# thisparticle/scl_slam

Measured on AMD Instinct MI355X. Metric: loop-closure candidates/sec: (scan, keyframe) pairs taken through full-database ARG-MIN detection per second (every pair aligned exactly and bounded by the f16 matrix-core screening; only the survivors get the f64 distance), batches of 16 scans, 10k-keyframe DB per GPU, higher is better.
Workload: dtype f64 results; f16-operand / f32-accumulate MFMA screening + f64 exact pass on the survivors

## Files before the change

### scl_slam_amd/csrc/engine.hip

```cpp
#include "scl_engine.h"

#include <hip/hip_runtime.h>

#include <cfloat>
#include <climits>
#include <chrono>
#include <cmath>
#include <cstdio>
#include <cstdlib>
#include <cstring>
#include <mutex>
#include <new>
#include <string>
#include <atomic>
#include <chrono>
#include <thread>
#include <vector>

#include "db_file.hpp"
#include "engine_internal.hpp"
#include "device_sort.hpp"
#include "plugin_host.hpp"

#ifdef SCL_DIAGNOSTICS
// ... 126 lines not shown
    dev_free(e->d_approx); dev_free(e->d_surv); dev_free(e->d_starts);
    size_t nn = n + n / 2 + 64;
    int rc;
    e->pair_cap = 0;
    if ((rc = dev_alloc(e, &e->d_approx, nn))) return rc;
    if ((rc = dev_alloc(e, &e->d_starts, nn))) return rc;
    if ((rc = dev_alloc(e, &e->d_surv, nn))) return rc;
    if ((rc = dev_alloc(e, &e->d_ring_d2, nn))) return rc;
    if ((rc = dev_alloc(e, &e->d_dist, nn))) return rc;
    if ((rc = dev_alloc(e, &e->d_shift, nn))) return rc;
    if ((rc = dev_alloc(e, &e->d_cand, nn))) return rc;
    e->pair_cap = nn;
    return SCL_OK;
}

int ensure_sets(scl_engine *e, size_t n)
{
    if (n <= e->set_stride && e->pair_cap >= e->set_stride * scl_engine::kScreenSets) return SCL_OK;
    const size_t stride = n + n / 4 + 64;
    int rc = ensure_pairs(e, stride * scl_engine::kScreenSets);
    if (rc) { e->set_stride = 0; return rc; }
    e->set_stride = stride;
    if (e->smask_cap < stride * scl_engine::kScreenSets) {
        dev_free(e->d_smask); e->d_smask = nullptr; e->smask_cap = 0;
        if ((rc = dev_alloc(e, &e->d_smask, stride * scl_engine::kScreenSets))) { e->set_stride = 0; return rc; }
        e->smask_cap = stride * scl_engine::kScreenSets;
    }
    const size_t need = 2 * stride * sc_screen_scratch_floats(db_view(e), e->SR);
    if (need > e->part_cap) {
        dev_free(e->d_part); e->part_cap = 0;
        if ((rc = dev_alloc(e, &e->d_part, need))) { e->set_stride = 0; return rc; }
        e->part_cap = need;
    }
    return SCL_OK;
}

int launch_topk(scl_engine *e, const QueryView &q, int lo, int hi, int k, float eps, hipStream_t on)
{
    hipStream_t s = on ? on : e->stream;
    ProfScope ps(e, P_TOPK, s);
    SCL_HIP(e, launch_ringkey_topk(db_view(e), q.rkey, lo, hi, k, eps, e->d_topk_scratch,
                                   e->d_topk_idx, e->d_topk_d2, s));
    return SCL_OK;
}

}

// ... 379 lines not shown
    if ((rc = dev_alloc(e, &e->d_done_counter, (size_t)4))) return bail(rc);
    if (hipMemset(e->d_done_counter, 0, 16) != hipSuccess) return bail(SCL_ERR_HIP);
    {
        constexpr int NS = scl_engine::kScreenSets;
        if ((rc = dev_alloc(e, &e->d_nsurv, (size_t)NS))) return bail(rc);
        static_assert(NS <= kTminEpsOffset, "the launch's largest bound sits kTminEpsOffset words behind its t_min word");
        if ((rc = dev_alloc(e, &e->d_tmin, (size_t)NS + kTminEpsOffset))) return bail(rc);
        if (hipMemset(e->d_nsurv, 0, sizeof(int) * NS) != hipSuccess) return bail(SCL_ERR_HIP);
        if (hipMemset(e->d_tmin, 0xff, sizeof(unsigned int) * NS) != hipSuccess) return bail(SCL_ERR_HIP);
        if (hipMemset(e->d_tmin + NS, 0, sizeof(unsigned int) * kTminEpsOffset) != hipSuccess) return bail(SCL_ERR_HIP);
        if ((rc = dev_alloc(e, &e->d_surv_part, (size_t)NS * kSurvivorBlocks * kTailRec))) return bail(rc);
        if ((rc = dev_alloc(e, &e->d_surv_done, (size_t)NS))) return bail(rc);
        if (hipMemset(e->d_surv_done, 0, sizeof(unsigned int) * NS) != hipSuccess) return bail(SCL_ERR_HIP);
        if (hipMalloc(&e->d_surv_args, (size_t)8 * NS * kSurvivorArgBytes) != hipSuccess) return bail(SCL_ERR_NOMEM);
        if (hipHostMalloc(&e->h_surv_args, (size_t)8 * NS * kSurvivorArgBytes, hipHostMallocDefault) != hipSuccess) return bail(SCL_ERR_HIP);
        if (hipHostMalloc((void **)&e->h_stream_out, (size_t)2 * NS * 64, hipHostMallocDefault) != hipSuccess) return bail(SCL_ERR_HIP);
        for (auto &ev : e->ev_chunk) if (hipEventCreateWithFlags(&ev, hipEventDisableTiming) != hipSuccess) return bail(SCL_ERR_HIP);
        for (auto &ev : e->ev_k1) if (hipEventCreateWithFlags(&ev, hipEventDisableTiming) != hipSuccess) return bail(SCL_ERR_HIP);
        for (auto &ev : e->ev_sub0) if (hipEventCreateWithFlags(&ev, hipEventDisableTiming) != hipSuccess) return bail(SCL_ERR_HIP);
        if (hipEventCreateWithFlags(&e->ev_align_gate, hipEventDisableTiming) != hipSuccess) return bail(SCL_ERR_HIP);
        {
            int lo_p = 0, hi_p = 0;
            (void)hipDeviceGetStreamPriorityRange(&lo_p, &hi_p);
            const bool wide_grid = e->S == 180 && e->RG == 20;
            if (hipStreamCreateWithPriority(&e->stream_surv, hipStreamNonBlocking, wide_grid ? hi_p : lo_p) != hipSuccess) return bail(SCL_ERR_HIP);
            if (hipStreamCreateWithPriority(&e->stream_queue_place, hipStreamNonBlocking, lo_p) != hipSuccess) return bail(SCL_ERR_HIP);
        }
    }
    if (hipStreamCreateWithFlags(&e->stream_alt, hipStreamNonBlocking) != hipSuccess) return bail(SCL_ERR_HIP);
    if (hipEventCreateWithFlags(&e->ev_db, hipEventDisableTiming) != hipSuccess) return bail(SCL_ERR_HIP);
// ... 49 lines not shown
    dev_free(e->d_smask);
    if (e->d_mat_dist) (void)hipFree(e->d_mat_dist);
    if (e->d_mat_shift) (void)hipFree(e->d_mat_shift);
    if (e->d_rank_key) (void)hipFree(e->d_rank_key);
    if (e->d_rank_pos) (void)hipFree(e->d_rank_pos);
    if (e->d_rank_out) (void)hipFree(e->d_rank_out);
    if (e->h_rank_out) (void)hipHostFree(e->h_rank_out);
    dev_free(e->d_meta_robot); dev_free(e->d_meta_index);
    if (e->h_mat) (void)hipHostFree(e->h_mat);
    for (auto &ev : e->ev_mat_k) if (ev) (void)hipEventDestroy(ev);
    for (auto &ev : e->ev_mat_c) if (ev) (void)hipEventDestroy(ev);
    dev_free(e->d_surv_stats);
    dev_free(e->d_surv_part); dev_free(e->d_surv_done);
    if (e->d_surv_args) (void)hipFree(e->d_surv_args);
    if (e->h_surv_args) (void)hipHostFree(e->h_surv_args);
    if (e->h_stream_out) (void)hipHostFree(e->h_stream_out);
    for (auto ev : e->ev_chunk) if (ev) (void)hipEventDestroy(ev);
    if (e->stream_surv) { (void)hipStreamSynchronize(e->stream_surv); (void)hipStreamDestroy(e->stream_surv); }
    if (e->stream_queue_place) (void)hipStreamDestroy(e->stream_queue_place);
    for (auto ev : e->ev_k1) if (ev) (void)hipEventDestroy(ev);
    for (auto ev : e->ev_sub0) if (ev) (void)hipEventDestroy(ev);
    if (e->ev_align_gate) (void)hipEventDestroy(e->ev_align_gate);
    dev_free(e->d_topk_scratch); dev_free(e->d_topk_idx); dev_free(e->d_topk_d2); dev_free(e->d_out3);
    dev_free(e->d_blk_part); dev_free(e->d_done_counter);
    if (e->ev_db) (void)hipEventDestroy(e->ev_db);
    if (e->stream_alt) { (void)hipStreamSynchronize(e->stream_alt); (void)hipStreamDestroy(e->stream_alt); }
    if (e->h_pinned) (void)hipHostFree(e->h_pinned);
    if (e->h_out3) (void)hipHostFree(e->h_out3);
    if (e->ev_call) (void)hipEventDestroy(e->ev_call);
    for (int i = 0; i < scl_engine::kSlots; ++i) if (e->ev_done[i]) (void)hipEventDestroy(e->ev_done[i]);
// ... 1538 lines not shown
```

### scl_slam_amd/csrc/engine_internal.hpp

```cpp
#pragma once

#include "scl_engine.h"

#include <hip/hip_runtime.h>

#include <chrono>
#include <climits>
#include <initializer_list>
#include <mutex>
#include <string>
#include <vector>

#include "icp.hpp"
#include "kernels.hpp"
#include "pcm.hpp"

namespace scl {

enum ProfKind { P_SC = 0, P_TOPK, P_ARGMIN, P_MAKESC, P_INGEST, P_ICPNN, P_ICPRED, P_COUNT };

struct PendingEvent { hipEvent_t start, stop; int kind; int launches = 1; };

struct ShardedFront;

// ... 39 lines not shown
    unsigned char *d_pbuf[3] = {nullptr, nullptr, nullptr}; size_t pbuf_cap = 0;
    static constexpr int kCopyStreams = 4;
    hipStream_t stream_copy = nullptr;
    hipStream_t stream_copy_x[kCopyStreams - 1] = {nullptr, nullptr, nullptr};
    hipEvent_t ev_copied[kCopyStreams][3] = {}, ev_consumed[3] = {nullptr, nullptr, nullptr};
    std::vector<void *> host_allocs;
    double *d_dist = nullptr; int *d_shift = nullptr; int *d_cand = nullptr; float *d_ring_d2 = nullptr; size_t pair_cap = 0;
#ifndef SCL_SCREEN_SETS
#define SCL_SCREEN_SETS 256
#endif
    static constexpr int kScreenSets = SCL_SCREEN_SETS;
    float *d_approx = nullptr; int *d_starts = nullptr; int *d_surv = nullptr;
    unsigned int *d_smask = nullptr; size_t smask_cap = 0;
    float *d_part = nullptr; size_t part_cap = 0;
    int *d_nsurv = nullptr; unsigned int *d_tmin = nullptr;
    unsigned long long *d_align_fallbacks = nullptr; uint64_t align_pairs = 0;
    unsigned long long *d_surv_stats = nullptr;
    size_t set_stride = 0;
    unsigned long long *d_surv_part = nullptr; unsigned int *d_surv_done = nullptr;
    void *d_surv_args = nullptr; void *h_surv_args = nullptr; unsigned surv_arg_tick = 0;
    double *h_stream_out = nullptr;
    hipEvent_t ev_chunk[2] = {nullptr, nullptr};
    bool exact_heavy = false;
    hipEvent_t ev_sub0[2] = {nullptr, nullptr};
    hipStream_t stream_surv = nullptr;
    hipEvent_t ev_k1[2] = {nullptr, nullptr};
    hipEvent_t ev_align_gate = nullptr;
    hipStream_t stream_queue_place = nullptr;
    bool screen = false;
    bool in_single_fallback = false;
// ... 43 lines not shown

struct ProfScope {
    scl_engine *e; int kind; hipStream_t s; hipEvent_t start = nullptr, stop = nullptr;
    ProfScope(scl_engine *e_, int kind_, hipStream_t s_ = nullptr);
    bool active() const { return start && stop; }
    ~ProfScope();
};
void collect_profile(scl_engine *e);
int sync(scl_engine *e);
hipError_t wait_event_polled(hipEvent_t ev, std::chrono::microseconds budget, bool relax);
void drain_keeping_error(scl_engine *e, const hipStream_t *streams, int n);
inline void drain_keeping_error(scl_engine *e, std::initializer_list<hipStream_t> streams) { drain_keeping_error(e, streams.begin(), (int)streams.size()); }
DbView db_view(const scl_engine *e);
int query_view(const scl_engine *e, int query, QueryView *q);
int ensure_pairs(scl_engine *e, size_t n);
int ensure_sets(scl_engine *e, size_t n);
int launch_topk(scl_engine *e, const QueryView &q, int lo, int hi, int k, float eps, hipStream_t on = nullptr);

template <class T> void dev_free(T *&p) { if (p) { (void)hipFree(p); p = nullptr; } }

constexpr int kQueryOutOfRange = -1, kQueryNotStaged = -2;
inline int query_slot(const scl_engine *e, int query, int n_db)
{
    if (query >= 0) return query < n_db ? query : kQueryOutOfRange;
    const int j = -1 - query;
    return j < e->stage_rows && e->staged[(size_t)j] ? e->cap + j : kQueryNotStaged;
}

inline int clamp_range(int &lo, int &hi, int n_db)
{
    if (lo < 0) lo = 0;
// ... 89 lines not shown
```

### scl_slam_amd/csrc/kernels.hpp

```cpp
#pragma once

#include <hip/hip_runtime.h>
#include <stdint.h>

#include <stdlib.h>

namespace scl {

#ifdef SCL_DIAGNOSTICS
inline int scl_lab_int(const char *name, int dflt) { const char *e = getenv(name); return e ? atoi(e) : dflt; }
inline bool scl_lab_is(const char *name, const char *value) { const char *e = getenv(name); if (!e) return false; while (*value) if (*e++ != *value++) return false; return true; }
#else
constexpr int scl_lab_int(const char *, int dflt) { return dflt; }
constexpr bool scl_lab_is(const char *, const char *) { return false; }
#endif

constexpr double kBigDist = 10000000.0;
constexpr int kTminEpsOffset = 256;
constexpr int hdesc_sector(int RG) { return ((RG * 8 + 63) / 64) * 8; }
constexpr int hkey_halfs(int S) { return ((S + 31) / 32) * 32; }
constexpr int hkey_store_halfs(int S) { return hkey_halfs(S) + 8; }
constexpr int hkey_row_halfs(int S) { return 2 * hkey_halfs(S) + 8; }
constexpr int halign_P(int S) { return S % 8 == 0 ? 8 : (S % 4 == 0 ? 4 : 0); }
constexpr int halign_CP(int S) { return ((S + 8 + 31) / 32) * 32; }
// ... 119 lines not shown
    int k; float exclude_eps; int *topk_idx; float *topk_d2;
    float *part;
    bool no_ring_metric;
};
bool sc_screen_supported(const struct DbView &db, int SR);
bool sc_screen_is_wide(const struct DbView &db, int SR);
float sc_screen_eps();
int sc_screen_max_batch(const struct DbView &db, int SR);
size_t sc_screen_scratch_floats(const struct DbView &db, int SR);
constexpr int kScreenAlign = 1, kScreenProducts = 2;
hipError_t launch_sc_screen_batch(const struct DbView &db, const ScreenBatch &sb, int SR, int align_filter, int num_cu, hipStream_t stream,
                                  int phases = kScreenAlign | kScreenProducts, const ScreenBatch *next = nullptr);
bool sc_screen_pairs(const struct DbView &db, int SR);
hipError_t launch_sc_screen_pair(const struct DbView &db, const ScreenBatch &sb0, const ScreenBatch &sb1, int SR, int align_filter, int num_cu,
                                 hipStream_t stream, const ScreenBatch *next0, const ScreenBatch *next1);
hipError_t launch_sc_select_batch(const ScreenBatch &sb, hipStream_t stream);
constexpr int kSurvivorBlocks = 2;
constexpr int kSurvivorArgBytes = 384;
constexpr int kMaxSurvivorQueries = 128;
struct SurvivorPass {
    int nq;
    int slot[kMaxSurvivorQueries], base[kMaxSurvivorQueries], n[kMaxSurvivorQueries], buf[kMaxSurvivorQueries];
    double *out3[kMaxSurvivorQueries];
    size_t pair_stride;
    const float *approx; int *survivors; unsigned int *t_min; double *out_dist; int *out_shift;
    const float *ring_d2; int k; float exclude_eps; int *topk_idx; float *topk_d2;
    unsigned long long *blk_part; unsigned int *done_counter;
    unsigned long long *surv_stats;
    void *d_args; void *h_args;
    int ring_from_keys;
// ... 62 lines not shown
```

### scl_slam_amd/csrc/sc_screen.hip

```cpp
#include <atomic>
#include <type_traits>

#include "align_exact.hpp"
#include "device_common.hpp"
#include "kernels.hpp"

namespace scl {

namespace {

typedef _Float16 h4 __attribute__((ext_vector_type(4)));
typedef _Float16 h8 __attribute__((ext_vector_type(8)));
typedef float f4v __attribute__((ext_vector_type(4)));
typedef float f2 __attribute__((ext_vector_type(2)));
typedef unsigned int u32x4 __attribute__((ext_vector_type(4)));
typedef u32x4 __attribute__((aligned(8))) u32x4_a8;

struct ScreenArgs {
    const double *vkey;
    const uint2 *hdesc; const unsigned int *kmask;
    const double *q_vkey; const float *q_rkey;
    const uint2 *q_hdesc; const unsigned int *q_kmask;
    const _Float16 *hkey; const _Float16 *q_hkey; int hkw;
    const float4 *rkey4; int rk_cap;
// ... 1738 lines not shown
            sc_align2_role<S, W>(ta.nb[0], ta.halign, ta.u_lo, ta.u_n, wg, wt, tile);
            sc_align2_role<S, W>(ta.nb[1], ta.halign, ta.u_lo, ta.u_n, wg, wt, tile);
        }
#endif
        else sc_align2_role<S, W>(ta.nb[0], ta.halign, ta.u_lo, ta.u_n, wg, wt, tile);
        return;
    }
    int qi, chunk;
    const int nq0 = ta.fin[0].prod.nq;
    if (!finish_block_of(b - ta.align_blocks, nq0 + ta.fin[1].prod.nq, ta.chunks_max, qi, chunk)) return;
    const int set = qi < nq0 ? 0 : 1;
    if (chunk >= ta.chunks[set]) return;
    sc_screen2_finish_body<RG, S, W, MASKS, D2>(ta.fin[set], qi - (set ? nq0 : 0), chunk);
}

static bool screen_second_form()
{
    static const int form = [] { const char *e = getenv("SCL_SCREEN_FORM"); return e ? atoi(e) : 2; }();
    return form != 1;
}
static bool screen_pair_enabled()
{
    static const int on = [] { const char *e = getenv("SCL_SCREEN_PAIR"); return e ? atoi(e) : 1; }();
    return on != 0;
}
static int screen_tail_pair()
{
    static const int v = [] { const char *e = getenv("SCL_TAIL_PAIR"); return e ? atoi(e) : 1; }();
    return v;
}
// ... 16 lines not shown
    ab->vkey = db.vkey; ab->rkey = db.rkey; ab->hdesc = db.hdesc; ab->kmask = db.kmask; ab->rkey4 = db.rkey4; ab->hkey = db.hkey; ab->hkw = hkey_row_halfs(db.S);
    ab->starts = sb.starts; ab->approx = sb.approx; ab->ring_d2 = sb.ring_d2; ab->t_min = sb.t_min; ab->fallbacks = sb.align_fallbacks; ab->smask = sb.smask;
    ab->pair_stride = (unsigned long long)sb.pair_stride;
    ab->S = db.S; ab->R4 = 4 * db.RG; ab->hstride = db.hstride; ab->rk_cap = db.cap; ab->align_filter = align_filter;
    ab->nq = sb.nq;
    int nmax = 0;
    for (int i = 0; i < sb.nq; ++i) {
        if (sb.n[i] <= 0) return -1;
        ab->q[i] = ScreenQuery{sb.slot[i], sb.base[i], sb.n[i], sb.buf[i]};
        nmax = sb.n[i] > nmax ? sb.n[i] : nmax;
    }
    for (int i = sb.nq; i < kMaxScreenBatch; ++i) ab->q[i] = ab->q[0];
    return nmax;
}

struct ScreenPairMate { const ScreenBatch *sb; const ScreenBatch *next; };

template <int RG, int S, int W, int OCC0, int OCC1>
static hipError_t launch_screen_grid(const DbView &db, const ScreenBatch &sb, int align_filter, int num_cu, hipStream_t stream, int phases,
                                     const ScreenBatch *next, const ScreenPairMate *mate = nullptr)
{
    constexpr int RGH = hdesc_rgh(RG);
    ScreenBatchArgs ab{};
    const int nmax = fill_screen_args(db, sb, align_filter, &ab);
    if (nmax < 0) return hipErrorInvalidValue;
    ScreenBatchArgs ab_m{};
    const int nmax_m = mate ? fill_screen_args(db, *mate->sb, align_filter, &ab_m) : 0;
    if (nmax_m < 0) return hipErrorInvalidValue;
    const int ngroups = (nmax + kGroup - 1) / kGroup;
    static_assert(halign_bytes(S) > 0, "alignment image");
    if (db.hstride != hdesc_stride(RG, S) || !sb.starts || !db.halign) return hipErrorInvalidValue;
// ... 97 lines not shown
                    if (e != hipSuccess) return e;
                    attrp.store(true, std::memory_order_release);
                }
                f2_m.prod = ab_m; f2_m.part = mate->sb->part; f2_m.nwg = nwg;
                union_of(*mate->sb, &f2_m.u_lo, &f2_m.u_n);
                Screen2PairArgs fp{};
                fp.prod[0] = ab; fp.prod[1] = ab_m; fp.part[0] = sb.part; fp.part[1] = mate->sb->part; fp.nwg = nwg;
                const int hi0 = f2.u_lo + f2.u_n, hi1 = f2_m.u_lo + f2_m.u_n;
                fp.u_lo = f2.u_lo < f2_m.u_lo ? f2.u_lo : f2_m.u_lo;
                fp.u_n = (hi0 > hi1 ? hi0 : hi1) - fp.u_lo;
                hipLaunchKernelGGL((sc_screen2_kernel<RG, S, W, 2>), dim3(nwg), dim3(S2Cfg<RG, S, W>::WV * kWave), (s2_lds<RG, S, W>()), stream, fp);
            }
        }
        if (!mate) hipLaunchKernelGGL((sc_screen2_kernel<RG, S, W>), dim3(nwg), dim3(S2Cfg<RG, S, W>::WV * kWave), (s2_lds<RG, S, W>()), stream, f2);
        if ((e = hipGetLastError()) != hipSuccess) return e;
        auto launch_tail = [&](const ScreenBatch &sb, const Screen2Args &f2, const int nmax, const ScreenBatch *next) -> hipError_t {
            const bool next_v2 = next && second_form_for(*next);
            const int chunks = (nmax + 255) / 256;
            const dim3 fgrid(finish_blocks(chunks, sb.nq)), ablock(kScreenWaves * kWave);
            if (!next) {
                hipLaunchKernelGGL((sc_screen2_finish_kernel<RG, S, W>), fgrid, dim3(256), 0, stream, f2, chunks);
                return hipGetLastError();
            }
            if (next->nq < 1 || next->nq > kMaxScreenBatch) return hipErrorInvalidValue;
            ScreenBatchArgs nb{};
            const int nmax2 = fill_screen_args(db, *next, align_filter, &nb);
            if (nmax2 < 0) return hipErrorInvalidValue;
            nb.skip_d2 = next_v2 ? 1 : 0;
            int ulo = 0, un = 0, ablocks;
            if (next_v2) {
// ... 94 lines not shown

bool sc_screen_pairs(const DbView &db, int SR)
{
    return sc_screen_supported(db, SR) && !sc_screen_is_wide(db, SR) && screen_second_form() && screen_pair_enabled() && screen_v2_min_env() <= kMaxScreenBatch &&
           scl_lab_int("SCL_SCREEN_VARIANT", 0) == 0 && scl_lab_int("SCL_SCREEN_PROBE", 0) == 0;
}

hipError_t launch_sc_screen_pair(const DbView &db, const ScreenBatch &sb0, const ScreenBatch &sb1, int SR, int align_filter, int num_cu, hipStream_t stream,
                                 const ScreenBatch *next0, const ScreenBatch *next1)
{
    if (!sc_screen_pairs(db, SR) || sb0.nq != kMaxScreenBatch || sb1.nq != kMaxScreenBatch) return hipErrorInvalidValue;
    const ScreenPairMate mate{&sb1, next1};
    return launch_screen_grid<16, 120, 13, 2, 3>(db, sb0, align_filter, num_cu, stream, kScreenProducts, next0, &mate);
}

}

#ifdef S2_STAMP
extern "C" int scl_debug_s2_stamps(unsigned long long *out)
{
    return (int)hipMemcpyFromSymbol(out, HIP_SYMBOL(scl::g_s2_stamps), sizeof(unsigned long long) * 4 * 64);
}
#endif
```

### scl_slam_amd/csrc/screen_host.hip

```cpp
#include "scl_engine.h"

#include <hip/hip_runtime.h>

#include <atomic>
#include <chrono>
#include <mutex>
#include <string>
#include <vector>

#include "engine_internal.hpp"
#include "plugin_host.hpp"
#include "screen_plan.hpp"

using namespace scl;

namespace {

int submit_full_many_locked(scl_engine *e, const int *queries, const int *los, const int *his, int nq, int *tickets);

void screen_batch_pointers(const scl_engine *e, ScreenBatch &sb, bool lists, unsigned long long *surv_stats, unsigned int *smask, float *part)
{
    sb.approx = e->d_approx; sb.starts = e->d_starts; sb.align_fallbacks = e->d_align_fallbacks; sb.ring_d2 = e->d_ring_d2;
    sb.survivors = lists ? e->d_surv : nullptr; sb.n_surv = lists ? e->d_nsurv : nullptr; sb.t_min = e->d_tmin; sb.surv_stats = surv_stats;
    sb.smask = smask; sb.part = part;
    sb.k = e->cfg.num_candidates; sb.exclude_eps = e->cfg.knn_exclude_eps; sb.topk_idx = e->d_topk_idx; sb.topk_d2 = e->d_topk_d2;
}

struct ScreenGroup { const int *qslot, *lo, *n; int nq, set0; int part_half = 0; bool masks = false; bool keys_later = false; };
void fill_screen_batch(scl_engine *e, ScreenBatch &sb, const ScreenGroup &g)
{
    sb.nq = g.nq;
    for (int j = 0; j < g.nq; ++j) { sb.slot[j] = g.qslot[j]; sb.base[j] = g.lo[j]; sb.n[j] = g.n[j]; sb.buf[j] = g.set0 + j; }
    sb.pair_stride = e->set_stride;
    screen_batch_pointers(e, sb, false, nullptr,
                          (g.masks || sc_screen_is_wide(db_view(e), e->SR)) ? e->d_smask : nullptr,
                          e->d_part + (g.part_half ? e->part_cap / 2 : 0));
    sb.no_ring_metric = g.keys_later;
}

int launch_screen_group(scl_engine *e, const ScreenGroup &cur, int phases = kScreenAlign | kScreenProducts,
                        const ScreenGroup *next = nullptr, hipStream_t stream = nullptr)
{
    if (!stream) stream = e->stream;
    ScreenBatch sb{}, nx{};
    fill_screen_batch(e, sb, cur);
    const bool has_next = next && next->nq > 0;
    if (has_next) fill_screen_batch(e, nx, *next);
    if (phases & kScreenAlign) for (int j = 0; j < cur.nq; ++j) e->align_pairs += (uint64_t)cur.n[j];
    if (has_next) for (int j = 0; j < next->nq; ++j) e->align_pairs += (uint64_t)next->n[j];
    if ((phases & kScreenAlign) && (phases & kScreenProducts) && has_next) {
        SCL_HIP(e, launch_sc_screen_batch(db_view(e), sb, e->SR, sc_align_filter_enabled(), e->num_cu, stream, kScreenAlign, nullptr));
// ... 11 lines not shown
    g0.part_half = 0; g1.part_half = 1;
    ScreenBatch sb0{}, sb1{}, nx0{}, nx1{};
    fill_screen_batch(e, sb0, g0);
    fill_screen_batch(e, sb1, g1);
    const bool has0 = next0 && next0->nq > 0, has1 = next1 && next1->nq > 0;
    if (has0) fill_screen_batch(e, nx0, *next0);
    if (has1) fill_screen_batch(e, nx1, *next1);
    const ScreenGroup *counted[4] = {align0 ? &g0 : nullptr, align1 ? &g1 : nullptr, has0 ? next0 : nullptr, has1 ? next1 : nullptr};
    for (const ScreenGroup *g : counted)
        if (g) for (int j = 0; j < g->nq; ++j) e->align_pairs += (uint64_t)g->n[j];
    if (align0) SCL_HIP(e, launch_sc_screen_batch(db_view(e), sb0, e->SR, sc_align_filter_enabled(), e->num_cu, stream, kScreenAlign, nullptr));
    if (align1) SCL_HIP(e, launch_sc_screen_batch(db_view(e), sb1, e->SR, sc_align_filter_enabled(), e->num_cu, stream, kScreenAlign, nullptr));
    ProfScope ps(e, P_SC, stream);
    SCL_HIP(e, launch_sc_screen_pair(db_view(e), sb0, sb1, e->SR, sc_align_filter_enabled(), e->num_cu, stream, has0 ? &nx0 : nullptr, has1 ? &nx1 : nullptr));
    if (ps.active()) { for (int j = 0; j < g0.nq; ++j) e->prof.sc_distance_pairs += (uint64_t)g0.n[j] + (uint64_t)g1.n[j]; }
    return SCL_OK;
}

unsigned survivor_arg_region(scl_engine *e) { return e->surv_arg_tick++ & 7u; }
int launch_survivor_pass(scl_engine *e, const int *qslot, const int *lo, const int *n, int nq, int set0, double *const *out3, hipStream_t stream = nullptr,
                         int phases = kSurvivorArgs | kSurvivorKernel, int region_in = -1, bool ring_from_keys = false)
{
    if (!stream) stream = e->stream;
    SurvivorPass sp{};
    sp.nq = nq; sp.ring_from_keys = ring_from_keys ? 1 : 0;
    for (int j = 0; j < nq; ++j) { sp.slot[j] = qslot[j]; sp.base[j] = lo[j]; sp.n[j] = n[j]; sp.buf[j] = set0 + j; sp.out3[j] = out3[j]; }
    sp.pair_stride = e->set_stride;
    sp.approx = e->d_approx; sp.survivors = e->d_surv; sp.t_min = e->d_tmin; sp.out_dist = e->d_dist; sp.out_shift = e->d_shift;
    sp.blk_part = e->d_surv_part; sp.done_counter = e->d_surv_done; sp.surv_stats = e->d_surv_stats;
    sp.ring_d2 = e->d_ring_d2; sp.k = e->cfg.num_candidates; sp.exclude_eps = e->cfg.knn_exclude_eps; sp.topk_idx = e->d_topk_idx; sp.topk_d2 = e->d_topk_d2;
// ... 371 lines not shown
    const int chmax = wide && CH > SCL_WIDE_CHUNK ? SCL_WIDE_CHUNK : CH;
    const int chn = spl >= 1 && spl <= chmax ? (chmax / spl) * spl : chmax;
    struct List { int qslot[CH], qlo[CH], qn[CH], pos[CH], m = 0; };
    struct Chunk { int first = 0, count = 0; int aligned = 0; bool busy = false, small = false; std::vector<int> lo, empty; };
    Chunk ch[2];
    bool sub0_valid[2] = {false, false};
    const bool small_exact = sc_small_exact_supported(db_view(e), e->SR) && (!wide || e->d_smask) && !scl_lab_is("SCL_STREAM_EXACT", "s");
    const bool keys_later = !wide && !small_exact;
    const bool pairs = !wide && sc_screen_pairs(db_view(e), e->SR);
    int nmax = 1;
    for (int i = 0; i < n_queries; ++i) {
        int l = lo[i], h = hi[i];
        const int n = clamp_range(l, h, n0);
        if (n > nmax) nmax = n;
    }
    int rc = ensure_sets(e, (size_t)nmax);
    if (rc) return rc;
    SCL_HIP(e, hipEventRecord(e->ev_align_gate, e->stream));
    SCL_HIP(e, hipStreamWaitEvent(e->stream_surv, e->ev_align_gate, 0));
    auto build = [&](int first, int count, List &L, Chunk *k) -> int {
        L.m = 0;
        for (int i = 0; i < count; ++i) {
            const int slot = query_slot(e, queries[first + i], n0);
            if (slot == kQueryOutOfRange) return fail(e, SCL_ERR_OUT_OF_RANGE, "query slot out of range");
            if (slot == kQueryNotStaged) return fail(e, SCL_ERR_INVALID_ARG, "no staged query");
            int l = lo[first + i], h = hi[first + i];
            const int n = clamp_range(l, h, n0);
            if (k) k->lo[(size_t)i] = l;
            if (n <= 0) continue;
            if (k) k->empty[(size_t)i] = 0;
            L.qslot[L.m] = slot; L.qlo[L.m] = l; L.qn[L.m] = n; L.pos[L.m] = i;
            ++L.m;
        }
        return SCL_OK;
    };
    auto submit = [&](int c, int first, int count, int nfirst, int ncount) -> int {
        Chunk &k = ch[c];
        k.first = first; k.count = count; k.lo.assign((size_t)count, 0); k.empty.assign((size_t)count, 1);
        List cur, nxt;
        if ((rc = build(first, count, cur, &k))) return rc;
        if (ncount > 0 && (rc = build(nfirst, ncount, nxt, nullptr))) return rc;
        double *out3[CH];
        for (int j = 0; j < cur.m; ++j) out3[j] = e->h_stream_out + ((size_t)c * NS + (size_t)cur.pos[j]) * 8;
        const int set0 = c * CH, nset0 = (c ^ 1) * CH;
        k.small = small_exact && !e->exact_heavy;
        const int region = (cur.m > 0 && (k.small || !wide)) ? (int)survivor_arg_region(e) : 0;
        if (cur.m > 0 && (k.small || !wide) && (rc = k.small ? launch_small_exact_chunk(e, cur.qslot, cur.qlo, cur.qn, cur.m, set0, out3, e->stream_surv, kSurvivorArgs, region)
                                                    : launch_survivor_pass(e, cur.qslot, cur.qlo, cur.qn, cur.m, set0, out3, e->stream_surv, kSurvivorArgs, region, keys_later))) return rc;
        if (ncount == 0 && cur.m > 0) SCL_HIP(e, hipEventRecord(e->ev_k1[c], e->stream_surv));
        struct ProfRestore { scl_engine *e; int saved; ~ProfRestore() { e->prof_on = saved; } } prof_restore{e, e->prof_on};
        hipEvent_t span_start = nullptr, span_stop = nullptr;
        int span_groups = 0;
        if (e->prof_on == 3 && cur.m > 0) {
            if ((e->prof_tick++ & 1) == 0) {
                auto get = [&]() { hipEvent_t ev = nullptr; if (!e->event_pool.empty()) { ev = e->event_pool.back(); e->event_pool.pop_back(); } else if (hipEventCreate(&ev) != hipSuccess) ev = nullptr; return ev; };
                span_start = get(); span_stop = get();
                if (span_start && span_stop) (void)hipEventRecord(span_start, e->stream); else { span_start = span_stop = nullptr; }
            }
            e->prof_on = 0;
        }
        auto span_end = [&]() {
            if (!span_start) return;
            (void)hipEventRecord(span_stop, e->stream);
            e->pending.push_back({span_start, span_stop, P_SC, span_groups});
            for (int j = 0; j < cur.m; ++j) e->prof.sc_distance_pairs += (uint64_t)cur.qn[j];
            span_start = nullptr;
        };
        static_assert(kPlanPairGroup == kMaxScreenBatch, "a pair is two full launch groups");
        PlanUnit units[CH];
        int next_aligned = 0;
        const int n_units = plan_chunk(cur.m, ncount > 0 ? nxt.m : 0, spl, pairs, k.aligned, units, &next_aligned);
        auto group_of = [&](const PlanGroup &p) {
            ScreenGroup g{nullptr, nullptr, nullptr, 0, 0};
            const int o = p.off - cur.m;
            if (p.nq > 0) g = o < 0 ? ScreenGroup{cur.qslot + p.off, cur.qlo + p.off, cur.qn + p.off, p.nq, set0 + p.off} : ScreenGroup{nxt.qslot + o, nxt.qlo + o, nxt.qn + o, p.nq, nset0 + o};
            g.keys_later = keys_later;
            return g;
        };
        for (int i = 0; i < n_units; ++i) {
            const PlanUnit &u = units[i];
            const ScreenGroup g0 = group_of(u.g0), g1 = group_of(u.g1), n0 = group_of(u.n0), n1 = group_of(u.n1);
            if (u.over > 0) {
                if (ch[c ^ 1].busy) SCL_HIP(e, hipStreamWaitEvent(e->stream, (wide && sub0_valid[c ^ 1] && u.over <= kWideExactBatch) ? e->ev_sub0[c ^ 1] : e->ev_chunk[c ^ 1], 0));
            }
            if (g1.nq > 0) rc = launch_screen_pair_group(e, g0, g1, u.align0, u.align1, n0.nq > 0 ? &n0 : nullptr, n1.nq > 0 ? &n1 : nullptr);
            else rc = launch_screen_group(e, g0, u.align0 ? (kScreenAlign | kScreenProducts) : kScreenProducts, n0.nq > 0 ? &n0 : nullptr);
            if (rc) return rc;
            ++span_groups;
        }
        span_end();
        hipStream_t xs = ncount > 0 ? e->stream_surv : e->stream;
        if (ncount > 0) {
            SCL_HIP(e, hipEventRecord(e->ev_k1[c], e->stream));
            SCL_HIP(e, hipStreamWaitEvent(e->stream_surv, e->ev_k1[c], 0));
        } else if (cur.m > 0) {
// ... 241 lines not shown
```

### scl_slam_amd/csrc/screen_plan.hpp

```cpp
#pragma once

namespace scl {

constexpr int kPlanPairGroup = 16;

struct PlanGroup { int off, nq; };

struct PlanUnit {
    PlanGroup g0, g1;
    PlanGroup n0, n1;
    bool align0, align1;
    int over;
};

inline int plan_chunk(int cur_m, int nxt_m, int spl, bool pairs, int aligned_in, PlanUnit *units, int *next_aligned)
{
    const int all_m = cur_m + nxt_m;
    auto group_at = [&](int off) {
        const int end = off < cur_m ? cur_m : all_m;
        if (off >= end) return PlanGroup{0, 0};
        return PlanGroup{off, end - off < spl ? end - off : spl};
    };
    auto pair_at = [&](int off) { return pairs && group_at(off).nq == kPlanPairGroup && group_at(off + kPlanPairGroup).nq == kPlanPairGroup &&
                                         (off + 2 * kPlanPairGroup <= cur_m || off >= cur_m); };
// ... 8 lines not shown
        if (end >= aligned_to) {
            u.n0 = group_at(end);
            if (pair && pair_at(end)) u.n1 = group_at(end + u.n0.nq);
        }
        const int reach = end + u.n0.nq + u.n1.nq;
        u.over = (reach > cur_m && u.n0.nq > 0) ? reach - cur_m : 0;
        u.align0 = g >= aligned_to;
        u.align1 = pair && g + u.g0.nq >= aligned_to;
        if (reach > aligned_to) aligned_to = reach;
        g = end;
    }
    *next_aligned = aligned_to > cur_m ? aligned_to - cur_m : 0;
    return n_units;
}

}
```

Measured before the change: 2.998 billion.

## Batch screen tails of several pair units into one joint run-tail launch

Adds a run planner that groups up to four consecutive full pair units. It launches only their products kernels, then fires a single tail kernel that does the finish work for all sets of the run plus the next groups' alignment. The tail arguments are staged into a ring of pinned host regions and copied on the survivor stream, gated by an event. The aim is fewer small tail launches and better CU fill in the finish and align phase. The cost is an extra partials scratch buffer per run, more host planning, and a cross-stream dependency on the argument copy.

```diff
diff --git a/scl_slam_amd/csrc/engine.hip b/scl_slam_amd/csrc/engine.hip
--- a/scl_slam_amd/csrc/engine.hip
+++ b/scl_slam_amd/csrc/engine.hip
@@ -164,10 +164,11 @@
     return SCL_OK;
 }
 
-int ensure_sets(scl_engine *e, size_t n)
-{
-    if (n <= e->set_stride && e->pair_cap >= e->set_stride * scl_engine::kScreenSets) return SCL_OK;
-    const size_t stride = n + n / 4 + 64;
+int ensure_sets(scl_engine *e, size_t n, int run_pairs)
+{
+    auto run_floats = [&](size_t stride) { return run_pairs > 1 ? (size_t)(2 * run_pairs) * stride * sc_screen_scratch_floats(db_view(e), e->SR) : (size_t)0; };
+    if (n <= e->set_stride && e->pair_cap >= e->set_stride * scl_engine::kScreenSets && e->part_run_cap >= run_floats(e->set_stride)) return SCL_OK;
+    const size_t stride = n <= e->set_stride ? e->set_stride : n + n / 4 + 64;
     int rc = ensure_pairs(e, stride * scl_engine::kScreenSets);
     if (rc) { e->set_stride = 0; return rc; }
     e->set_stride = stride;
@@ -181,6 +182,11 @@
         dev_free(e->d_part); e->part_cap = 0;
         if ((rc = dev_alloc(e, &e->d_part, need))) { e->set_stride = 0; return rc; }
         e->part_cap = need;
+    }
+    if (run_floats(stride) > e->part_run_cap) {
+        dev_free(e->d_part_run); e->part_run_cap = 0;
+        if ((rc = dev_alloc(e, &e->d_part_run, run_floats(stride)))) { e->set_stride = 0; return rc; }
+        e->part_run_cap = run_floats(stride);
     }
     return SCL_OK;
 }
@@ -590,6 +596,9 @@
         if (hipMemset(e->d_surv_done, 0, sizeof(unsigned int) * NS) != hipSuccess) return bail(SCL_ERR_HIP);
         if (hipMalloc(&e->d_surv_args, (size_t)8 * NS * kSurvivorArgBytes) != hipSuccess) return bail(SCL_ERR_NOMEM);
         if (hipHostMalloc(&e->h_surv_args, (size_t)8 * NS * kSurvivorArgBytes, hipHostMallocDefault) != hipSuccess) return bail(SCL_ERR_HIP);
+        if (hipMalloc(&e->d_run_args, (size_t)scl_engine::kRunArgRegions * kScreenRunArgBytes) != hipSuccess) return bail(SCL_ERR_NOMEM);
+        if (hipHostMalloc(&e->h_run_args, (size_t)scl_engine::kRunArgRegions * kScreenRunArgBytes, hipHostMallocDefault) != hipSuccess) return bail(SCL_ERR_HIP);
+        for (auto &ev : e->ev_run_args) if (hipEventCreateWithFlags(&ev, hipEventDisableTiming) != hipSuccess) return bail(SCL_ERR_HIP);
         if (hipHostMalloc((void **)&e->h_stream_out, (size_t)2 * NS * 64, hipHostMallocDefault) != hipSuccess) return bail(SCL_ERR_HIP);
         for (auto &ev : e->ev_chunk) if (hipEventCreateWithFlags(&ev, hipEventDisableTiming) != hipSuccess) return bail(SCL_ERR_HIP);
         for (auto &ev : e->ev_k1) if (hipEventCreateWithFlags(&ev, hipEventDisableTiming) != hipSuccess) return bail(SCL_ERR_HIP);
@@ -669,6 +678,10 @@
     dev_free(e->d_surv_part); dev_free(e->d_surv_done);
     if (e->d_surv_args) (void)hipFree(e->d_surv_args);
     if (e->h_surv_args) (void)hipHostFree(e->h_surv_args);
+    dev_free(e->d_part_run);
+    if (e->d_run_args) (void)hipFree(e->d_run_args);
+    if (e->h_run_args) (void)hipHostFree(e->h_run_args);
+    for (auto &ev : e->ev_run_args) if (ev) (void)hipEventDestroy(ev);
     if (e->h_stream_out) (void)hipHostFree(e->h_stream_out);
     for (auto ev : e->ev_chunk) if (ev) (void)hipEventDestroy(ev);
     if (e->stream_surv) { (void)hipStreamSynchronize(e->stream_surv); (void)hipStreamDestroy(e->stream_surv); }
diff --git a/scl_slam_amd/csrc/engine_internal.hpp b/scl_slam_amd/csrc/engine_internal.hpp
--- a/scl_slam_amd/csrc/engine_internal.hpp
+++ b/scl_slam_amd/csrc/engine_internal.hpp
@@ -77,6 +77,10 @@
     unsigned int *d_smask = nullptr; size_t smask_cap = 0;
     float *d_part = nullptr; size_t part_cap = 0;
     int *d_nsurv = nullptr; unsigned int *d_tmin = nullptr;
+    float *d_part_run = nullptr; size_t part_run_cap = 0;
+    static constexpr int kRunArgRegions = 16;
+    void *d_run_args = nullptr; void *h_run_args = nullptr; unsigned run_arg_tick = 0;
+    hipEvent_t ev_run_args[2] = {nullptr, nullptr};
     unsigned long long *d_align_fallbacks = nullptr; uint64_t align_pairs = 0;
     unsigned long long *d_surv_stats = nullptr;
     size_t set_stride = 0;
@@ -150,7 +154,7 @@
 DbView db_view(const scl_engine *e);
 int query_view(const scl_engine *e, int query, QueryView *q);
 int ensure_pairs(scl_engine *e, size_t n);
-int ensure_sets(scl_engine *e, size_t n);
+int ensure_sets(scl_engine *e, size_t n, int run_pairs = 1);
 int launch_topk(scl_engine *e, const QueryView &q, int lo, int hi, int k, float eps, hipStream_t on = nullptr);
 
 template <class T> void dev_free(T *&p) { if (p) { (void)hipFree(p); p = nullptr; } }
diff --git a/scl_slam_amd/csrc/kernels.hpp b/scl_slam_amd/csrc/kernels.hpp
--- a/scl_slam_amd/csrc/kernels.hpp
+++ b/scl_slam_amd/csrc/kernels.hpp
@@ -157,6 +157,14 @@
 bool sc_screen_pairs(const struct DbView &db, int SR);
 hipError_t launch_sc_screen_pair(const struct DbView &db, const ScreenBatch &sb0, const ScreenBatch &sb1, int SR, int align_filter, int num_cu,
                                  hipStream_t stream, const ScreenBatch *next0, const ScreenBatch *next1);
+constexpr int kScreenRunPairs = 4, kScreenRunSets = 2 * kScreenRunPairs;
+constexpr size_t kScreenRunArgBytes = 12 * 1024;
+int sc_screen_tail_run(const struct DbView &db, int SR);
+hipError_t launch_sc_screen_pair_products(const struct DbView &db, const ScreenBatch &sb0, const ScreenBatch &sb1, int SR, int align_filter, int num_cu,
+                                          hipStream_t stream);
+struct ScreenRunTail { int n_fin, n_al; const ScreenBatch *fin[kScreenRunSets]; const ScreenBatch *al[kScreenRunSets]; };
+hipError_t fill_sc_screen_run_tail(const struct DbView &db, const ScreenRunTail &rt, int SR, int align_filter, int num_cu, void *h_args, unsigned int *grid);
+hipError_t launch_sc_screen_run_tail(const void *d_args, unsigned int grid, hipStream_t stream);
 hipError_t launch_sc_select_batch(const ScreenBatch &sb, hipStream_t stream);
 constexpr int kSurvivorBlocks = 2;
 constexpr int kSurvivorArgBytes = 384;
diff --git a/scl_slam_amd/csrc/sc_screen.hip b/scl_slam_amd/csrc/sc_screen.hip
--- a/scl_slam_amd/csrc/sc_screen.hip
+++ b/scl_slam_amd/csrc/sc_screen.hip
@@ -1,4 +1,5 @@
 #include <atomic>
+#include <new>
 #include <type_traits>
 
 #include "align_exact.hpp"
@@ -1776,6 +1777,43 @@
     sc_screen2_finish_body<RG, S, W, MASKS, D2>(ta.fin[set], qi - (set ? nq0 : 0), chunk);
 }
 
+struct TailRunArgs {
+    Screen2Args fin[kScreenRunSets];
+    ScreenBatchArgs nb[kScreenRunSets];
+    const unsigned char *halign;
+    int n_fin_scans;
+    int chunks[kScreenRunSets], chunks_max;
+    int n_items;
+    int u_lo[kScreenRunPairs], u_n[kScreenRunPairs], ablocks[kScreenRunPairs];
+    int align_blocks;
+};
+static_assert(sizeof(TailRunArgs) <= kScreenRunArgBytes, "argument region of a run's tail");
+
+template <int RG, int S, int W, bool MASKS, bool D2>
+__global__ __launch_bounds__(kScreenWaves * kWave, 3) void sc_screen2_tail_run_kernel(const TailRunArgs *__restrict__ ta_global)
+{
+    extern __shared__ __attribute__((aligned(16))) unsigned char smem_tailr[];
+    typedef const TailRunArgs __attribute__((address_space(4))) *ConstArgs;
+    const ConstArgs ta = (ConstArgs)ta_global;
+    const int b = (int)blockIdx.x;
+    const int align_blocks = ta->align_blocks;
+    if (b < align_blocks) {
+        const int n_items = ta->n_items;
+        const int s = b >> 3, r = s / n_items, item = s - r * n_items, wb = 8 * r + (b & 7);
+        const int ab = ta->ablocks[item];
+        if (wb >= ab) return;
+        const int wave = __builtin_amdgcn_readfirstlane((int)(threadIdx.x >> 6));
+        sc_align2_pair_role<S, W>((const ScreenBatchArgs *)(ta->nb + 2 * item), ta->halign, ta->u_lo[item], ta->u_n[item], wb * kScreenWaves + wave, ab * kScreenWaves,
+                                  smem_tailr + (size_t)wave * Align2Cfg<S>::LDS_WAVE);
+        return;
+    }
+    int qi, chunk;
+    if (!finish_block_of(b - align_blocks, ta->n_fin_scans, ta->chunks_max, qi, chunk)) return;
+    const int set = qi / kMaxScreenBatch;
+    if (chunk >= ta->chunks[set]) return;
+    sc_screen2_finish_body<RG, S, W, MASKS, D2>(*(const Screen2Args *)(ta->fin + set), qi - set * kMaxScreenBatch, chunk);
+}
+
 static bool screen_second_form()
 {
     static const int form = [] { const char *e = getenv("SCL_SCREEN_FORM"); return e ? atoi(e) : 2; }();
@@ -1822,7 +1860,7 @@
     return nmax;
 }
 
-struct ScreenPairMate { const ScreenBatch *sb; const ScreenBatch *next; };
+struct ScreenPairMate { const ScreenBatch *sb; const ScreenBatch *next; bool products_only = false; };
 
 template <int RG, int S, int W, int OCC0, int OCC1>
 static hipError_t launch_screen_grid(const DbView &db, const ScreenBatch &sb, int align_filter, int num_cu, hipStream_t stream, int phases,
@@ -1950,6 +1988,7 @@
         }
         if (!mate) hipLaunchKernelGGL((sc_screen2_kernel<RG, S, W>), dim3(nwg), dim3(S2Cfg<RG, S, W>::WV * kWave), (s2_lds<RG, S, W>()), stream, f2);
         if ((e = hipGetLastError()) != hipSuccess) return e;
+        if (mate && mate->products_only) return hipSuccess;
         auto launch_tail = [&](const ScreenBatch &sb, const Screen2Args &f2, const int nmax, const ScreenBatch *next) -> hipError_t {
             const bool next_v2 = next && second_form_for(*next);
             const int chunks = (nmax + 255) / 256;
@@ -2074,6 +2113,88 @@
     return launch_screen_grid<16, 120, 13, 2, 3>(db, sb0, align_filter, num_cu, stream, kScreenProducts, next0, &mate);
 }
 
+static int screen_tail_run_env()
+{
+    static const int v = [] { const char *e = getenv("SCL_TAIL_RUN"); const int k = e ? atoi(e) : 1; return k >= 4 ? 4 : k >= 2 ? 2 : 1; }();
+    return v;
+}
+int sc_screen_tail_run(const DbView &db, int SR)
+{
+    return (sc_screen_pairs(db, SR) && screen_tail_pair() == 1) ? screen_tail_run_env() : 1;
+}
+
+hipError_t launch_sc_screen_pair_products(const DbView &db, const ScreenBatch &sb0, const ScreenBatch &sb1, int SR, int align_filter, int num_cu, hipStream_t stream)
+{
+    if (!sc_screen_pairs(db, SR) || sb0.nq != kMaxScreenBatch || sb1.nq != kMaxScreenBatch) return hipErrorInvalidValue;
+    ScreenPairMate mate{&sb1, nullptr};
+    mate.products_only = true;
+    return launch_screen_grid<16, 120, 13, 2, 3>(db, sb0, align_filter, num_cu, stream, kScreenProducts, nullptr, &mate);
+}
+
+hipError_t fill_sc_screen_run_tail(const DbView &db, const ScreenRunTail &rt, int SR, int align_filter, int num_cu, void *h_args, unsigned int *grid)
+{
+    constexpr int RG = 16, S = 120, W = 13;
+    if (sc_screen_tail_run(db, SR) < 2 || !h_args || !grid || !db.halign || rt.n_fin < 2 || rt.n_fin > kScreenRunSets || (rt.n_fin & 1) ||
+        rt.n_al < 0 || rt.n_al > kScreenRunSets || (rt.n_al & 1)) return hipErrorInvalidValue;
+    auto full = [](const ScreenBatch *b) { return b && b->nq == kMaxScreenBatch && b->part && !b->smask && !b->no_ring_metric; };
+    auto union_of = [](const ScreenBatch &b, int *lo_out, int *hi_out) {
+        int lo = b.base[0], hi = b.base[0] + b.n[0];
+        for (int i = 1; i < b.nq; ++i) { lo = b.base[i] < lo ? b.base[i] : lo; hi = b.base[i] + b.n[i] > hi ? b.base[i] + b.n[i] : hi; }
+        *lo_out = lo; *hi_out = hi;
+    };
+    TailRunArgs *ta = new (h_args) TailRunArgs{};
+    ta->halign = db.halign;
+    int nwg = (num_cu / (16 * S2Cfg<RG, S, W>::NP)) * (16 * S2Cfg<RG, S, W>::NP);
+    if (nwg < 16 * S2Cfg<RG, S, W>::NP) nwg = 16 * S2Cfg<RG, S, W>::NP;
+    for (int s = 0; s < rt.n_fin; ++s) {
+        if (!full(rt.fin[s])) return hipErrorInvalidValue;
+        Screen2Args &f2 = ta->fin[s];
+        const int nmax = fill_screen_args(db, *rt.fin[s], align_filter, &f2.prod);
+        if (nmax < 0) return hipErrorInvalidValue;
+        f2.prod.skip_d2 = 1;
+        f2.part = rt.fin[s]->part; f2.nwg = nwg;
+        int lo, hi;
+        union_of(*rt.fin[s], &lo, &hi);
+        f2.u_lo = lo; f2.u_n = hi - lo;
+        ta->chunks[s] = (nmax + 255) / 256;
+        ta->chunks_max = ta->chunks[s] > ta->chunks_max ? ta->chunks[s] : ta->chunks_max;
+    }
+    ta->n_fin_scans = rt.n_fin * kMaxScreenBatch;
+    ta->n_items = rt.n_al / 2;
+    static const int wgs_env = scl_lab_int("SCL_ALIGN2_WGS", 0);
+    int amax = 0;
+    for (int i = 0; i < ta->n_items; ++i) {
+        int lo = 0, hi = 0;
+        for (int s = 2 * i; s < 2 * i + 2; ++s) {
+            if (!rt.al[s] || rt.al[s]->nq != kMaxScreenBatch) return hipErrorInvalidValue;
+            if (fill_screen_args(db, *rt.al[s], align_filter, &ta->nb[s]) < 0) return hipErrorInvalidValue;
+            ta->nb[s].skip_d2 = 1;
+            int l, h;
+            union_of(*rt.al[s], &l, &h);
+            if (s == 2 * i) { lo = l; hi = h; } else { lo = l < lo ? l : lo; hi = h > hi ? h : hi; }
+        }
+        ta->u_lo[i] = lo; ta->u_n[i] = hi - lo;
+        int b = (ta->u_n[i] + kScreenWaves * 3 - 1) / (kScreenWaves * 3);
+        int cap = (wgs_env > 0 ? wgs_env : 2 * num_cu) / ta->n_items;
+        cap = cap < 1 ? 1 : cap;
+        b = b > cap ? cap : b;
+        ta->ablocks[i] = b < 1 ? 1 : b;
+        amax = ta->ablocks[i] > amax ? ta->ablocks[i] : amax;
+    }
+    ta->align_blocks = 8 * ((amax + 7) / 8) * ta->n_items;
+    *grid = (unsigned int)(ta->align_blocks + finish_blocks(ta->chunks_max, ta->n_fin_scans));
+    return hipSuccess;
+}
+
+hipError_t launch_sc_screen_run_tail(const void *d_args, unsigned int grid, hipStream_t stream)
+{
+    constexpr size_t lds_a2 = (size_t)kScreenWaves * Align2Cfg<120>::LDS_WAVE;
+    if (!d_args || grid < 1) return hipErrorInvalidValue;
+    hipLaunchKernelGGL((sc_screen2_tail_run_kernel<16, 120, 13, false, true>), dim3(grid), dim3(kScreenWaves * kWave), lds_a2, stream,
+                       static_cast<const TailRunArgs *>(d_args));
+    return hipGetLastError();
+}
+
 }
 
 #ifdef S2_STAMP
diff --git a/scl_slam_amd/csrc/screen_host.hip b/scl_slam_amd/csrc/screen_host.hip
--- a/scl_slam_amd/csrc/screen_host.hip
+++ b/scl_slam_amd/csrc/screen_host.hip
@@ -26,7 +26,7 @@
     sb.k = e->cfg.num_candidates; sb.exclude_eps = e->cfg.knn_exclude_eps; sb.topk_idx = e->d_topk_idx; sb.topk_d2 = e->d_topk_d2;
 }
 
-struct ScreenGroup { const int *qslot, *lo, *n; int nq, set0; int part_half = 0; bool masks = false; bool keys_later = false; };
+struct ScreenGroup { const int *qslot, *lo, *n; int nq, set0; int part_half = 0; bool masks = false; bool keys_later = false; float *part = nullptr; };
 void fill_screen_batch(scl_engine *e, ScreenBatch &sb, const ScreenGroup &g)
 {
     sb.nq = g.nq;
@@ -34,7 +34,7 @@
     sb.pair_stride = e->set_stride;
     screen_batch_pointers(e, sb, false, nullptr,
                           (g.masks || sc_screen_is_wide(db_view(e), e->SR)) ? e->d_smask : nullptr,
-                          e->d_part + (g.part_half ? e->part_cap / 2 : 0));
+                          g.part ? g.part : e->d_part + (g.part_half ? e->part_cap / 2 : 0));
     sb.no_ring_metric = g.keys_later;
 }
 
@@ -76,6 +76,57 @@
     ProfScope ps(e, P_SC, stream);
     SCL_HIP(e, launch_sc_screen_pair(db_view(e), sb0, sb1, e->SR, sc_align_filter_enabled(), e->num_cu, stream, has0 ? &nx0 : nullptr, has1 ? &nx1 : nullptr));
     if (ps.active()) { for (int j = 0; j < g0.nq; ++j) e->prof.sc_distance_pairs += (uint64_t)g0.n[j] + (uint64_t)g1.n[j]; }
+    return SCL_OK;
+}
+
+struct RunTail { const void *d_args = nullptr; unsigned int grid = 0; };
+size_t run_part_floats(const scl_engine *e) { return e->set_stride * sc_screen_scratch_floats(db_view(e), e->SR); }
+int stage_run_tail(scl_engine *e, const ScreenGroup *fin, int n_fin, const ScreenGroup *al, int n_al, hipStream_t copy_stream, RunTail *out)
+{
+    ScreenBatch fb[kScreenRunSets], ab[kScreenRunSets];
+    ScreenRunTail rt{};
+    rt.n_fin = n_fin; rt.n_al = n_al;
+    for (int j = 0; j < n_fin; ++j) {
+        ScreenGroup g = fin[j];
+        g.part = e->d_part_run + (size_t)j * run_part_floats(e);
+        fb[j] = ScreenBatch{};
+        fill_screen_batch(e, fb[j], g);
+        rt.fin[j] = &fb[j];
+    }
+    for (int j = 0; j < n_al; ++j) {
+        ab[j] = ScreenBatch{};
+        fill_screen_batch(e, ab[j], al[j]);
+        rt.al[j] = &ab[j];
+        for (int i = 0; i < al[j].nq; ++i) e->align_pairs += (uint64_t)al[j].n[i];
+    }
+    const size_t region = (size_t)(e->run_arg_tick++ % (unsigned)scl_engine::kRunArgRegions) * kScreenRunArgBytes;
+    char *h = static_cast<char *>(e->h_run_args) + region, *d = static_cast<char *>(e->d_run_args) + region;
+    SCL_HIP(e, fill_sc_screen_run_tail(db_view(e), rt, e->SR, sc_align_filter_enabled(), e->num_cu, h, &out->grid));
+    SCL_HIP(e, hipMemcpyAsync(d, h, kScreenRunArgBytes, hipMemcpyHostToDevice, copy_stream));
+    out->d_args = d;
+    return SCL_OK;
+}
+
+int launch_screen_run_unit(scl_engine *e, ScreenGroup g0, ScreenGroup g1, int j, bool align0, bool align1, const RunTail *tail, hipEvent_t wait_for)
+{
+    hipStream_t stream = e->stream;
+    g0.part = e->d_part_run + (size_t)(2 * j) * run_part_floats(e);
+    g1.part = e->d_part_run + (size_t)(2 * j + 1) * run_part_floats(e);
+    ScreenBatch sb0{}, sb1{};
+    fill_screen_batch(e, sb0, g0);
+    fill_screen_batch(e, sb1, g1);
+    const ScreenGroup *counted[2] = {align0 ? &g0 : nullptr, align1 ? &g1 : nullptr};
+    for (const ScreenGroup *g : counted)
+        if (g) for (int i = 0; i < g->nq; ++i) e->align_pairs += (uint64_t)g->n[i];
+    if (align0) SCL_HIP(e, launch_sc_screen_batch(db_view(e), sb0, e->SR, sc_align_filter_enabled(), e->num_cu, stream, kScreenAlign, nullptr));
+    if (align1) SCL_HIP(e, launch_sc_screen_batch(db_view(e), sb1, e->SR, sc_align_filter_enabled(), e->num_cu, stream, kScreenAlign, nullptr));
+    ProfScope ps(e, P_SC, stream);
+    SCL_HIP(e, launch_sc_screen_pair_products(db_view(e), sb0, sb1, e->SR, sc_align_filter_enabled(), e->num_cu, stream));
+    if (tail) {
+        if (wait_for) SCL_HIP(e, hipStreamWaitEvent(stream, wait_for, 0));
+        SCL_HIP(e, launch_sc_screen_run_tail(tail->d_args, tail->grid, stream));
+    }
+    if (ps.active()) { for (int i = 0; i < g0.nq; ++i) e->prof.sc_distance_pairs += (uint64_t)g0.n[i] + (uint64_t)g1.n[i]; }
     return SCL_OK;
 }
 
@@ -477,7 +528,8 @@
         const int n = clamp_range(l, h, n0);
         if (n > nmax) nmax = n;
     }
-    int rc = ensure_sets(e, (size_t)nmax);
+    const int run_pairs = (pairs && !keys_later) ? sc_screen_tail_run(db_view(e), e->SR) : 1;
+    int rc = ensure_sets(e, (size_t)nmax, run_pairs);
     if (rc) return rc;
     SCL_HIP(e, hipEventRecord(e->ev_align_gate, e->stream));
     SCL_HIP(e, hipStreamWaitEvent(e->stream_surv, e->ev_align_gate, 0));
@@ -506,6 +558,29 @@
         double *out3[CH];
         for (int j = 0; j < cur.m; ++j) out3[j] = e->h_stream_out + ((size_t)c * NS + (size_t)cur.pos[j]) * 8;
         const int set0 = c * CH, nset0 = (c ^ 1) * CH;
+        static_assert(kPlanPairGroup == kMaxScreenBatch && kPlanRunPairs == kScreenRunPairs, "a pair is two full launch groups; a run's tail takes kScreenRunPairs pairs");
+        PlanUnit units[CH];
+        PlanRun runs[CH];
+        int next_aligned = 0, n_runs = 0;
+        (void)plan_chunk_runs(cur.m, ncount > 0 ? nxt.m : 0, spl, pairs, run_pairs, k.aligned, units, runs, &n_runs, &next_aligned);
+        auto group_of = [&](const PlanGroup &p) {
+            ScreenGroup g{nullptr, nullptr, nullptr, 0, 0};
+            const int o = p.off - cur.m;
+            if (p.nq > 0) g = o < 0 ? ScreenGroup{cur.qslot + p.off, cur.qlo + p.off, cur.qn + p.off, p.nq, set0 + p.off} : ScreenGroup{nxt.qslot + o, nxt.qlo + o, nxt.qn + o, p.nq, nset0 + o};
+            g.keys_later = keys_later;
+            return g;
+        };
+        RunTail run_tail[CH / (2 * kMaxScreenBatch) + 1];
+        bool any_tail = false;
+        for (int r = 0, t = 0; r < n_runs; ++r) {
+            if (!runs[r].joint) continue;
+            ScreenGroup fin[kScreenRunSets], al[kScreenRunSets];
+            for (int j = 0; j < runs[r].n_fin; ++j) fin[j] = group_of(runs[r].fin[j]);
+            for (int j = 0; j < runs[r].n_al; ++j) al[j] = group_of(runs[r].al[j]);
+            if ((rc = stage_run_tail(e, fin, runs[r].n_fin, al, runs[r].n_al, e->stream_surv, &run_tail[t++]))) return rc;
+            any_tail = true;
+        }
+        if (any_tail) SCL_HIP(e, hipEventRecord(e->ev_run_args[c], e->stream_surv));
         k.small = small_exact && !e->exact_heavy;
         const int region = (cur.m > 0 && (k.small || !wide)) ? (int)survivor_arg_region(e) : 0;
         if (cur.m > 0 && (k.small || !wide) && (rc = k.small ? launch_small_exact_chunk(e, cur.qslot, cur.qlo, cur.qn, cur.m, set0, out3, e->stream_surv, kSurvivorArgs, region)
@@ -529,19 +604,20 @@
             for (int j = 0; j < cur.m; ++j) e->prof.sc_distance_pairs += (uint64_t)cur.qn[j];
             span_start = nullptr;
         };
-        static_assert(kPlanPairGroup == kMaxScreenBatch, "a pair is two full launch groups");
-        PlanUnit units[CH];
-        int next_aligned = 0;
-        const int n_units = plan_chunk(cur.m, ncount > 0 ? nxt.m : 0, spl, pairs, k.aligned, units, &next_aligned);
-        auto group_of = [&](const PlanGroup &p) {
-            ScreenGroup g{nullptr, nullptr, nullptr, 0, 0};
-            const int o = p.off - cur.m;
-            if (p.nq > 0) g = o < 0 ? ScreenGroup{cur.qslot + p.off, cur.qlo + p.off, cur.qn + p.off, p.nq, set0 + p.off} : ScreenGroup{nxt.qslot + o, nxt.qlo + o, nxt.qn + o, p.nq, nset0 + o};
-            g.keys_later = keys_later;
-            return g;
-        };
-        for (int i = 0; i < n_units; ++i) {
-            const PlanUnit &u = units[i];
+        for (int r = 0, t = 0; r < n_runs; ++r) {
+            if (runs[r].joint) {
+                const RunTail &tail = run_tail[t++];
+                for (int j = 0; j < runs[r].nu; ++j) {
+                    const PlanUnit &u = units[runs[r].u0 + j];
+                    const bool last_unit = j == runs[r].nu - 1;
+                    hipEvent_t wait_for = nullptr;
+                    if (last_unit && ((runs[r].over > 0 && ch[c ^ 1].busy) || hipEventQuery(e->ev_run_args[c]) != hipSuccess)) wait_for = e->ev_run_args[c];
+                    if ((rc = launch_screen_run_unit(e, group_of(u.g0), group_of(u.g1), j, u.align0, u.align1, last_unit ? &tail : nullptr, wait_for))) return rc;
+                    ++span_groups;
+                }
+                continue;
+            }
+            const PlanUnit &u = units[runs[r].u0];
             const ScreenGroup g0 = group_of(u.g0), g1 = group_of(u.g1), n0 = group_of(u.n0), n1 = group_of(u.n1);
             if (u.over > 0) {
                 if (ch[c ^ 1].busy) SCL_HIP(e, hipStreamWaitEvent(e->stream, (wide && sub0_valid[c ^ 1] && u.over <= kWideExactBatch) ? e->ev_sub0[c ^ 1] : e->ev_chunk[c ^ 1], 0));
diff --git a/scl_slam_amd/csrc/screen_plan.hpp b/scl_slam_amd/csrc/screen_plan.hpp
--- a/scl_slam_amd/csrc/screen_plan.hpp
+++ b/scl_slam_amd/csrc/screen_plan.hpp
@@ -46,4 +46,81 @@
     return n_units;
 }
 
+constexpr int kPlanRunPairs = 4;
+constexpr int kPlanRunGroups = 2 * kPlanRunPairs;
+
+struct PlanRun {
+    int u0, nu;
+    bool joint;
+    int n_fin, n_al;
+    PlanGroup fin[kPlanRunGroups];
+    PlanGroup al[kPlanRunGroups];
+    int over;
+};
+
+inline int plan_chunk_runs(int cur_m, int nxt_m, int spl, bool pairs, int run_pairs, int aligned_in, PlanUnit *units, PlanRun *runs, int *n_runs,
+                           int *next_aligned)
+{
+    if (run_pairs <= 1 || !pairs) {
+        const int n_units = plan_chunk(cur_m, nxt_m, spl, pairs, aligned_in, units, next_aligned);
+        for (int i = 0; i < n_units; ++i) { runs[i] = PlanRun{}; runs[i].u0 = i; runs[i].nu = 1; runs[i].joint = false; runs[i].over = units[i].over; }
+        *n_runs = n_units;
+        return n_units;
+    }
+    if (run_pairs > kPlanRunPairs) run_pairs = kPlanRunPairs;
+    const int all_m = cur_m + nxt_m;
+    constexpr int PG = kPlanPairGroup;
+    auto group_at = [&](int off) {
+        const int end = off < cur_m ? cur_m : all_m;
+        if (off >= end) return PlanGroup{0, 0};
+        return PlanGroup{off, end - off < spl ? end - off : spl};
+    };
+    auto pair_at = [&](int off) { return group_at(off).nq == PG && group_at(off + PG).nq == PG && (off + 2 * PG <= cur_m || off >= cur_m); };
+    int n_units = 0, nr = 0, aligned_to = aligned_in;
+    for (int g = 0; g < cur_m;) {
+        PlanRun &r = runs[nr++];
+        r = PlanRun{};
+        r.u0 = n_units;
+        if (!pair_at(g)) {
+            PlanUnit &u = units[n_units++];
+            u.g0 = group_at(g); u.g1 = PlanGroup{0, 0};
+            const int end = g + u.g0.nq;
+            u.n0 = u.n1 = PlanGroup{0, 0};
+            if (end >= aligned_to) u.n0 = group_at(end);
+            const int reach = end + u.n0.nq;
+            u.over = (reach > cur_m && u.n0.nq > 0) ? reach - cur_m : 0;
+            u.align0 = g >= aligned_to; u.align1 = false;
+            if (reach > aligned_to) aligned_to = reach;
+            r.nu = 1; r.joint = false; r.over = u.over;
+            g = end;
+            continue;
+        }
+        int nu = 1;
+        while (nu < run_pairs && g + 2 * PG * nu < cur_m && pair_at(g + 2 * PG * nu) && g + 2 * PG * (nu + 1) <= aligned_to) ++nu;
+        for (int j = 0; j < nu; ++j) {
+            PlanUnit &u = units[n_units++];
+            const int o = g + 2 * PG * j;
+            u.g0 = group_at(o); u.g1 = group_at(o + PG);
+            u.n0 = u.n1 = PlanGroup{0, 0};
+            u.over = 0;
+            u.align0 = o >= aligned_to; u.align1 = o + PG >= aligned_to;
+            r.fin[r.n_fin++] = u.g0; r.fin[r.n_fin++] = u.g1;
+        }
+        const int end = g + 2 * PG * nu;
+        int reach = end;
+        if (end >= aligned_to)
+            while (r.n_al < 2 * run_pairs && pair_at(reach) && (reach < cur_m) == (end < cur_m)) {
+                r.al[r.n_al++] = group_at(reach); r.al[r.n_al++] = group_at(reach + PG);
+                reach += 2 * PG;
+            }
+        r.nu = nu; r.joint = true;
+        r.over = (reach > cur_m && r.n_al > 0) ? reach - cur_m : 0;
+        if (reach > aligned_to) aligned_to = reach;
+        g = end;
+    }
+    *n_runs = nr;
+    *next_aligned = aligned_to > cur_m ? aligned_to - cur_m : 0;
+    return n_units;
 }
+
+}
```

Result: no change. 3.004 billion (median of 2 runs) (+0.2%).
